# hlz0606/DH-AUG-DH-Forward-Kinematics-Model-Driven-Augmentation-for-3D-Human-Pose-Estimation

Measured on AMD Instinct MI355X. Metric: augmented poses/sec (FK+GAN step), 16-joint batch=65536, higher is better.
Workload: dtype bf16; 1 GPU; FK+Gen+D3+D2 forward; batch_per_gpu=65536, frames=1, global_batch=65536, dense_dim=256, preAngle=True, fk_dtype=f32, dense_dtype=bf16 MFMA, fp32 accumulate

## Files before the change

dh-aug-dh-forward-kinematics-model-driven-augmentation-for-3d-human-pose-estimation_amd/_lib.py:

```python
import ctypes
import os

_HERE = os.path.dirname(os.path.abspath(__file__))
LIB_PATH = os.environ.get("DHAUG_LIB", os.path.join(_HERE, "lib", "libdhaug.so"))

_vp, _i64, _i32, _f32 = ctypes.c_void_p, ctypes.c_int64, ctypes.c_int, ctypes.c_float
_u64 = ctypes.c_uint64

SIGNATURES = {
    "dhaug_fk_forward": [_vp, _vp, _vp, _vp, _i64, _i32, _vp],
    "dhaug_fk_backward": [_vp, _vp, _vp, _vp, _vp, _vp, _i64, _vp],
    "dhaug_gen_tail_forward": [_vp, _vp, _vp, _vp, _vp, _i64, _i32, _vp],
    "dhaug_gen_tail_forward_critics": [_vp, _vp, _vp, _vp, _vp, _vp, _vp, _vp, _vp, _vp, _i32, _u64, _u64, _vp, _i64, _i32, _i32, _vp],
    "dhaug_gen_tail_backward": [_vp, _vp, _vp, _vp, _vp, _i64, _i32, _vp],
    "dhaug_bone_length": [_vp, _vp, _i64, _vp],
    "dhaug_kcs_forward": [_vp, _vp, _vp, _i64, _i64, _i32, _vp],
    "dhaug_center_kcs_forward": [_vp, _vp, _vp, _i64, _i64, _i32, _vp],
    "dhaug_kcs_backward": [_vp, _vp, _vp, _i64, _i32, _vp],
    "dhaug_kcs_jvp": [_vp, _vp, _vp, _i64, _i32, _vp],
    "dhaug_world_to_camera_project": [_vp, _vp, _vp, _vp, _vp, _vp, _i64, _vp],
    "dhaug_world_to_camera_project_backward": [_vp, _vp, _vp, _vp, _vp, _vp, _vp, _i64, _vp],
    "dhaug_camera_to_world": [_vp, _vp, _vp, _vp, _i64, _vp],
    "dhaug_bone_length_swap": [_vp, _vp, _vp, _i64, _vp],
    "dhaug_project_to_2d": [_vp, _vp, _vp, _i64, _vp],
# ... 93 lines not shown
class AdamDesc(ctypes.Structure):
    _fields_ = [("off", _i64), ("len", _i64), ("nt", _vp), ("N", _i32), ("K", _i32), ("Kp", _i32), ("pad_", _i32), ("item0", _i64)]


class TnLayer(ctypes.Structure):
    _fields_ = [("A", _vp), ("lda", _i64), ("B", _vp), ("ldb", _i64), ("C", _vp), ("ldc", _i64), ("colsum_a", _vp),
                ("colsum_rows", _i64), ("M", _i64), ("N1", _i32), ("N2", _i32), ("accumulate", _i32), ("max_workgroups", _i32),
                ("planes_a", _i32), ("planes_b", _i32)]


class Block2(ctypes.Structure):
    _fields_ = [("W1", _vp), ("ldw1", _i64), ("W2", _vp), ("ldw2", _i64), ("bits1", _vp), ("bits2", _vp), ("Y1", _vp), ("ldy1", _i64),
                ("Y2", _vp), ("ldy2", _i64)]


class TopDesc(ctypes.Structure):
    _fields_ = [("seed", _vp), ("ld_seed", _i64), ("wout", _vp), ("ld_wout", _i64), ("x", _vp), ("ldx", _i64), ("m1", _vp), ("mh", _vp),
                ("m0", _vp), ("ld_m", _i64), ("w2", _vp), ("ldw2", _i64), ("w1", _vp), ("ldw1", _i64), ("wm", _vp), ("ldwm", _i64),
                ("bits0", _vp), ("bits1", _vp), ("g2", _vp), ("g1", _vp), ("g0", _vp), ("ld_g", _i64), ("gcat", _vp), ("ld_gcat", _i64),
                ("M", _i64), ("n0", _i64), ("nc", _i64), ("mask_act", _i32), ("mask_slope", _f32)]


SIGNATURES["dhaug_critic_top_backward_bf16"] = [ctypes.POINTER(TopDesc), _vp]
SIGNATURES["dhaug_critic_top_tangent_bf16"] = [ctypes.POINTER(TopDesc), _vp]
BLOCK2_MAX = 3
SIGNATURES["dhaug_gemm_block2_stack_bf16"] = [_vp, _i64, ctypes.POINTER(Block2), _i32, _i32, _f32, _i64, _vp]
TN_GROUP_MAX = 42
TN_GROUP_WORKSPACE_FLOATS = 256 * (256 * 256 + 256)
SIGNATURES["dhaug_gemm_tn_group_bf16"] = [ctypes.POINTER(TnLayer), _i32, _vp, _vp]
SIGNATURES["dhaug_pack_wfrag"] = [_vp, _i64, _vp, _i64, _i64, _i64, _vp]
SIGNATURES["dhaug_pack_wfrag_batch"] = [_vp, _i32, _vp]
SIGNATURES["dhaug_pack_wfrag_composed"] = [_vp, _i64, _vp, _vp, _i64, _vp, _vp, _vp, _i64, _i64, _i64, _i64, _vp]
SIGNATURES["dhaug_mlp_forward"] = [ctypes.POINTER(MlpUnit), _i32, _i64, _vp]
SIGNATURES["dhaug_pack_wfrag_f16x2"] = [_vp, _i64, _vp, _i64, _i64, _i64, _vp]
SIGNATURES["dhaug_pack_wfrag_f16x2_t16"] = [_vp, _i64, _vp, _i64, _i64, _i64, _vp]
SIGNATURES["dhaug_mlp_forward_x3"] = [ctypes.POINTER(MlpUnit), _i32, _i64, _vp]

EVAL_MAX_THRESHOLDS = 32
EVAL_MAX_MULTIPLICITY = 1024
EVAL_TOTALS_WORDS = 3 + EVAL_MAX_THRESHOLDS
EVAL_WORKSPACE_BYTES = 2048 * EVAL_TOTALS_WORDS * 8
LOSS_METER_WORDS = 3
POSETRAIN_WORKSPACE_BYTES = 2048 * 8

ERRORS = {-1: "DHAUG_EINVAL (bad argument)", -2: "DHAUG_EALIGN (alignment contract violated)",
          -3: "DHAUG_EUNSUPPORTED (shape not implemented)"}

_lib = None


def lib():
    global _lib
    if _lib is None:
        if not os.path.exists(LIB_PATH):
            raise RuntimeError("libdhaug.so not found at %s: build it with `python __graft_entry__.py build` "
                               "(there is no fallback path)" % LIB_PATH)
        L = ctypes.CDLL(LIB_PATH)
        L.dhaug_version.restype = ctypes.c_int
        L.dhaug_arch.restype = ctypes.c_char_p
        for name, args in SIGNATURES.items():
            fn = getattr(L, name)
            fn.argtypes = args
            fn.restype = ctypes.c_int
        if os.environ.get("DHAUG_NAN_PROPAGATION", "") in ("1", "true", "yes"):
            L.dhaug_set_nan_propagation(1)
        _lib = L
# ... 21 lines not shown
```

dh-aug-dh-forward-kinematics-model-driven-augmentation-for-3d-human-pose-estimation_amd/csrc/dhaug_mlp.hip:

```cpp
#include <cstdlib>
#include "dhaug_common.h"

namespace {

typedef short bf16x8 __attribute__((ext_vector_type(8)));
typedef short bf16x4 __attribute__((ext_vector_type(4)));
typedef float f32x16 __attribute__((ext_vector_type(16)));
typedef float f32x4 __attribute__((ext_vector_type(4)));

constexpr int MLP_BM = 128;
constexpr int MLP_MT = MLP_BM / 32;
constexpr int MLP_THREADS = 256;
constexpr int MLP_NS = 2;
constexpr int MLP_MAX_UNITS = 32;
constexpr int MLP_MAX_KSTEPS = 16;
constexpr int BUF01_PITCH = 256, BUF2_PITCH = 128;
constexpr int BUF01_BYTES = MLP_BM * BUF01_PITCH * 2;
constexpr int BUF2_BYTES = MLP_BM * BUF2_PITCH * 2;
constexpr int MLP_LDS_BYTES = 2 * BUF01_BYTES + BUF2_BYTES;

enum { U_LOAD_F32 = 0, U_LOAD_BF16 = 1, U_STORE_BF16 = 2, U_GEMM = 3 };
#if (defined(DHAUG_MLP_SAVE_TU) || defined(DHAUG_MLP_NAN_SAFE)) && !defined(SAVE_ABL_NONANSAFE)
constexpr bool NAN_SAFE_TU = true;
#else
constexpr bool NAN_SAFE_TU = false;
#endif
enum { F_OUT_F32 = 4, F_DOT_OUT = 16 };

struct Unit {
    int kind;
    int plan;
    int flags;
    int src, dst, res;
    int src2, ksteps2;
    int ksteps, N, act;
    float slope;
    int cols;
    long long ld;
    const void* g;
    const uint16_t* w;
    const uint16_t* w2;
    const float* bias;
    uint16_t* save;
    long long save_ld;
    long long save_rows;
    uint32_t* bits;
};
enum { PLAN_STACK = 1 << 13, PLAN_LEAKY = 1 << 10, PLAN_ALT = 1 << 11, PLAN_TAIL = 1 << 12, PLAN_TAIL_BF16 = 1 << 14, PLAN_OUT = 1 << 28,
       PLAN_DOT = 1 << 29, PLAN_PAIR = 1 << 30 };

struct Program {
    int nunits;
    int min_run;
    Unit u[MLP_MAX_UNITS];
};

__device__ __forceinline__ unsigned char* buf_base(unsigned char* smem, int id) {
    return smem + (id == 0 ? 0 : (id == 1 ? BUF01_BYTES : 2 * BUF01_BYTES));
}
__device__ __forceinline__ int buf_pitch_bytes(int id) { return (id == 2 ? BUF2_PITCH : BUF01_PITCH) * 2; }
__device__ __forceinline__ int chunk_off(int row, int c, int pitch_bytes) { return row * pitch_bytes + ((c ^ (row & 15)) << 4); }

__device__ __forceinline__ float act_neg(int act, float slope) {
    return act == DHAUG_ACT_RELU ? 0.0f : (act == DHAUG_ACT_LRELU ? slope : 1.0f);
}
__device__ __forceinline__ float act_fn(float v, float neg) { return fmaxf(v, v * neg); }
typedef __bf16 bf16v2 __attribute__((ext_vector_type(2)));
typedef float f32v2 __attribute__((ext_vector_type(2)));
__device__ __forceinline__ uint32_t pack_bf16x2(float a, float b) {
    f32v2 f = {a, b};
    return __builtin_bit_cast(uint32_t, __builtin_convertvector(f, bf16v2));
}

typedef short s16x2_t __attribute__((ext_vector_type(2)));
typedef uint32_t u32x4_t __attribute__((ext_vector_type(4)));
__device__ __forceinline__ uint32_t pk_relu(uint32_t packed, uint32_t lb) {
    return __builtin_bit_cast(uint32_t, __builtin_elementwise_max(__builtin_bit_cast(s16x2_t, packed), __builtin_bit_cast(s16x2_t, lb)));
}

constexpr int MLP_CH = 4;
constexpr int OUT_PITCH = 68;
typedef const Unit __attribute__((address_space(4))) * UnitPtr;
// ... 501 lines not shown
                        }
                        if (BITS && k == KS - 1) bits_store(mt - 1);
                    }
                }
                __builtin_amdgcn_sched_barrier(0);
            }
        }
        if (RESMODE == 1 || (RESMODE == 2 && has_res)) {
#pragma unroll
            for (int i = 0; i < 4; ++i) {
                acc[mt & 1][i & 1] = __builtin_amdgcn_mfma_f32_32x32x16_bf16(idl[i >> 1], rx[2 * (i & 1) + (i >> 1)], acc[mt & 1][i & 1], 0, 0, 0);
            }
            __builtin_amdgcn_sched_barrier(0);
        }
        DHAUG_LSTAMP(dbg + 1 + mt)
        DHAUG_BB_SPLIT()
    }
    if (!LEAD) quad_store(MLP_MT - 2, 28, st0, st1);
#pragma unroll
    for (int j = 0; j < 32; j += 4) {
        const uint32_t p0 = pair_pack(acc[(MLP_MT - 1) & 1], j), p1 = pair_pack(acc[(MLP_MT - 1) & 1], j + 2);
        quad_store(MLP_MT - 1, j, p0, p1);
        if (BITS) {
            bits_or(p0, j >> 1);
            bits_or(p1, (j >> 1) + 1);
        }
    }
    if (BITS) bits_store(MLP_MT - 1);
    DHAUG_LSTAMP(dbg + 5)
#pragma unroll
    for (int t = 0; t < MLP_NS; ++t) seed[t] = nseed[t];
}

__device__ __forceinline__ void tail_layer(const StackDesc& d, unsigned char* smem, int wave, int lane, const WHalf& wlo,
                                           const WHalf& whi, const f32x16 (&seed)[MLP_NS]) {
    constexpr int TILE_BYTES = 32 * BUF01_PITCH * 2;
    const int r31 = lane & 31, h = lane >> 5, x = lane & 15;
    const unsigned char* src = buf_base(smem, d.src) + wave * TILE_BYTES;
    float* st = reinterpret_cast<float*>(buf_base(smem, d.dst)) + (32 * wave + r31) * OUT_PITCH + 4 * h;
    const float neg = act_neg(d.act, d.slope);
    const int lfx = r31 * (BUF01_PITCH * 2) | ((x >> 1) << 5) | ((h ^ (x & 1)) << 4);
    bf16x8 fx[4];
#pragma unroll
    for (int k = 0; k < 3; ++k) fx[k] = *reinterpret_cast<const bf16x8*>(src + (lfx ^ (k << 5)));
    f32x16 acc[MLP_NS];
#pragma unroll
    for (int k = 0; k < MLP_MAX_KSTEPS; ++k) {
        if (k + 3 < MLP_MAX_KSTEPS) fx[(k + 3) & 3] = *reinterpret_cast<const bf16x8*>(src + (lfx ^ ((k + 3) << 5)));
#pragma unroll
        for (int t = 0; t < MLP_NS; ++t)
            acc[t] = __builtin_amdgcn_mfma_f32_32x32x16_bf16(k < 8 ? wlo[t][k & 7] : whi[t][k & 7], fx[k & 3],
                                                             k == 0 ? seed[t] : acc[t], 0, 0, 0);
    }
#pragma unroll
    for (int t = 0; t < MLP_NS; ++t)
#pragma unroll
        for (int g = 0; g < 4; ++g) {
            f32x4 v;
#pragma unroll
            for (int e = 0; e < 4; ++e) v[e] = act_fn(acc[t][4 * g + e], neg);
            *reinterpret_cast<f32x4*>(st + 32 * t + 8 * g) = v;
        }
}

__device__ __forceinline__ void tail_gemm(const StackDesc& d, unsigned char* smem, int wave, int lane, const WHalf& wlo,
                                          const WHalf& whi, const f32x16 (&seed)[MLP_NS]) {
// ... 63 lines not shown
                o.x = pack_bf16x2(act_fn(acc[mt][4 * g + 0], neg), act_fn(acc[mt][4 * g + 1], neg));
                o.y = pack_bf16x2(act_fn(acc[mt][4 * g + 2], neg), act_fn(acc[mt][4 * g + 3], neg));
                *reinterpret_cast<uint2*>(dst + chunk_off(32 * mt + r31, 4 * wave + g, pbd) + (h << 3)) = o;
            }
    }
}

struct Sweep {
    int row, c, dr, dc, q;
    __device__ __forceinline__ Sweep(int tid, int q_) : q(q_) {
        row = tid / q_; c = tid - row * q_; dr = MLP_THREADS / q_; dc = MLP_THREADS - dr * q_;
    }
    __device__ __forceinline__ void next() {
        row += dr; c += dc;
        if (c >= q) { c -= q; ++row; }
    }
};

__device__ __forceinline__ void save_image(int id, uint16_t* g, long long ld, int cols, unsigned char* smem, long long m0, long long M,
                                           int tid) {
    asm volatile("" : "+v"(tid));
#if defined(SAVE_ABL_NOSTORE)
    return;
#endif
    const unsigned char* img = buf_base(smem, id);
    const int pb = buf_pitch_bytes(id);
    for (Sweep sw(tid, cols >> 3); sw.row < MLP_BM; sw.next())
        if (m0 + sw.row < M)
            *reinterpret_cast<uint4*>(g + (m0 + sw.row) * ld + sw.c * 8) = *reinterpret_cast<const uint4*>(img + chunk_off(sw.row, sw.c, pb));
}

template <bool LEAKY, bool ALT, bool SAVE>
__device__ __forceinline__ void gemm_stack(UnitPtr lead, int lead_ks, UnitPtr first, int n, int tail, unsigned char* smem,
                                           int wave, int lane, long long m0, long long M, int tid) {
    (void)tid;
    auto save_of = [&](UnitPtr su, bool on, int& ld_bytes) -> __amdgpu_buffer_rsrc_t {
        uint16_t* base = (SAVE && on) ? su->save : nullptr;
        long long ld = (SAVE && on) ? su->save_ld : 0;
        const long long lim = (SAVE && on) ? su->save_rows : 0;
        long long rows = lim - m0 < MLP_BM ? lim - m0 : MLP_BM;
        if (rows <= 0) { rows = 0; ld = 0; base = nullptr; }
        ld_bytes = (int)(ld * 2);
#if defined(SAVE_ABL_NOSTORE) || defined(SAVE_ABL_NULLSTORES)
        base = nullptr;
#endif
        return __builtin_amdgcn_make_buffer_rsrc(base != nullptr ? base + m0 * ld : reinterpret_cast<uint16_t*>(smem), 0,
                                                 base != nullptr ? (int)(rows * ld * 2) : 0, 0x27000);
    };
    auto bits_of = [&](UnitPtr bu) -> __amdgpu_buffer_rsrc_t {
        uint32_t* base = SAVE ? bu->bits : nullptr;
        return __builtin_amdgcn_make_buffer_rsrc(base != nullptr ? base + (m0 / MLP_BM) * 1024 : reinterpret_cast<uint32_t*>(smem), 0,
                                                 base != nullptr ? 4096 : 0, 0x27000);
    };
    const int nt = n + (tail ? 1 : 0);
    StackDesc cur = stack_desc(first), nxt = stack_desc(first + (nt > 1 ? 1 : 0));
    WHalf loA, loB, hi;
    f32x16 seed[MLP_NS];
    bf16x8 idf[2];
#pragma unroll
    for (int ks2 = 0; ks2 < 2; ++ks2) {
        const int dd = (lane & 31) - 16 * ks2 - 8 * (lane >> 5);
        u32x4 v;
#pragma unroll
        for (int p2 = 0; p2 < 4; ++p2) v[p2] = (dd == 2 * p2 ? 0x3F80u : 0u) | (dd == 2 * p2 + 1 ? 0x3F800000u : 0u);
        idf[ks2] = __builtin_bit_cast(bf16x8, v);
    }
    int nold = 0;
    const __amdgpu_buffer_rsrc_t nosv = save_of(first, false, nold);
    if (lead_ks != 0) {
        const StackDesc ld = stack_desc(lead);
        load_seed(ld.bias, wave, 4, lane, seed);
        if (lead_ks == 8) {
            const WBase<8> b(ld.w, wave, 4, lane);
#pragma unroll
            for (int t = 0; t < MLP_NS; ++t)
#pragma unroll
                for (int k = 0; k < 8; ++k) loB[t][k] = b.frag(t, k);
            stack_layer<LEAKY, 0, 8, false, SAVE>(ld, cur, smem, wave, lane, loB, loA, hi, seed, idf, MLP_MAX_UNITS + 50, nosv, 0, bits_of(lead));
        } else {
            const WBase<4> b(ld.w, wave, 4, lane);
#pragma unroll
            for (int t = 0; t < MLP_NS; ++t)
#pragma unroll
                for (int k = 0; k < 4; ++k) loB[t][k] = b.frag(t, k);
            stack_layer<LEAKY, 0, 4, false, SAVE>(ld, cur, smem, wave, lane, loB, loA, hi, seed, idf, MLP_MAX_UNITS + 50, nosv, 0, bits_of(lead));
        }
        lds_barrier();
        DHAUG_LSTAMP(MLP_MAX_UNITS + 56)
    } else {
        load_seed(cur.bias, wave, 4, lane, seed);
        const WBase<> b0(cur.w, wave, 4, lane);
#pragma unroll
        for (int t = 0; t < MLP_NS; ++t)
#pragma unroll
            for (int k = 0; k < MLP_MAX_KSTEPS / 2; ++k) {
                loA[t][k] = b0.frag(t, k);
                hi[t][k] = b0.frag(t, k + 8);
            }
    }
    int l = 0;
#pragma unroll 1
    for (; l + 2 <= n; l += 2) {
// ... 247 lines not shown
    for (int i = 0; i < 2 * nw; ++i) s += st[i * MLP_BM + tid];
    static_cast<float*>(const_cast<void*>(u->g))[(m0 + tid) * u->ld] = s;
}

__device__ __forceinline__ void store_output(UnitPtr u, unsigned char* smem, long long m0, long long M, int tid) {
    const float* st = reinterpret_cast<const float*>(buf_base(smem, u->dst));
    float* out = static_cast<float*>(const_cast<void*>(u->g));
    const long long ld = u->ld;
    for (Sweep sw(tid, u->N); sw.row < MLP_BM; sw.next())
        if (m0 + sw.row < M) out[(m0 + sw.row) * ld + sw.c] = st[sw.row * OUT_PITCH + sw.c];
}

template <bool SAVE>
__global__ __launch_bounds__(MLP_THREADS, 1) void fused_mlp_kernel(Program prog, long long M) {
    extern __shared__ __attribute__((aligned(16))) unsigned char smem[];
    const int tid = threadIdx.x, lane = tid & 63;
    const int wave = __builtin_amdgcn_readfirstlane(tid >> 6);
    const long long ntiles = (M + MLP_BM - 1) / MLP_BM;
    const unsigned char __attribute__((address_space(4)))* ka =
        (const unsigned char __attribute__((address_space(4)))*)__builtin_amdgcn_kernarg_segment_ptr();
    UnitPtr units = (UnitPtr)(ka + __builtin_offsetof(Program, u));
    const int nunits = *(const int __attribute__((address_space(4)))*)(ka + __builtin_offsetof(Program, nunits));
    int hk = units->kind, hp = units->plan;
    for (long long tile = blockIdx.x; tile < ntiles; tile += gridDim.x) {
        const long long m0 = tile * MLP_BM;
        int i = 0;
#pragma unroll 1
        while (i < nunits) {
            UnitPtr u = units + i;
            const int kind = hk, plan = hp;
            int ni = i + 1;
            if (kind == U_GEMM && (plan & PLAN_STACK)) ni = i + ((plan & 15) != 0) + ((plan >> 4) & 63) + ((plan & (PLAN_TAIL | PLAN_TAIL_BF16)) ? 1 : 0);
            if (kind == U_GEMM && (plan & PLAN_PAIR)) ni = i + 2;
            {
                UnitPtr nu = units + (ni < nunits ? ni : 0);
                hk = nu->kind;
                hp = nu->plan;
            }
            DHAUG_STAMP(i)
            DHAUG_LSTAMP(MLP_MAX_UNITS + 64 + 4 * i)
            const int ui = i;
            i = ni;
            (void)ui;
            if (kind != U_GEMM) {
                if (kind == U_LOAD_BF16 && (plan & 1)) __syncthreads();
                move_unit(u, smem, m0, M, tid);
                if (kind == U_STORE_BF16) {
                    lds_barrier();
                    continue;
                }
            } else {
                if (plan & PLAN_STACK) {
                    const int lead_ks = plan & 15, run = (plan >> 4) & 63;
                    const int tail = (plan & PLAN_TAIL) ? 1 : ((plan & PLAN_TAIL_BF16) ? 2 : 0);
                    UnitPtr f0 = u + (lead_ks != 0), tu = f0 + run;
                    if ((plan & PLAN_LEAKY) || NAN_SAFE_TU) gemm_stack<true, false, SAVE>(u, lead_ks, f0, run, tail, smem, wave, lane, m0, M, tid);
                    else if (plan & PLAN_ALT) gemm_stack<false, true, SAVE>(u, lead_ks, f0, run, tail, smem, wave, lane, m0, M, tid);
                    else gemm_stack<false, false, SAVE>(u, lead_ks, f0, run, tail, smem, wave, lane, m0, M, tid);
                    lds_barrier();
                    if (SAVE) {
                        UnitPtr lu = tu - 1;
                        if (lu->save != nullptr) save_image(lu->dst, lu->save, lu->save_ld, (lu->N + 15) & ~15, smem, m0, lu->save_rows, tid);
                        if (tail == 2 && tu->save != nullptr)
                            save_image(tu->dst, tu->save, tu->save_ld, (tu->N + 15) & ~15, smem, m0, tu->save_rows, tid);
                    }
                    if (tail == 1) {
                        store_output(tu, smem, m0, M, tid);
                        lds_barrier();
                    }

                    continue;
                }
                const int nslices = (plan >> 24) & 15, dbg = MLP_MAX_UNITS + 64 + 4 * ui;
                if (plan & PLAN_PAIR) {
                    gemm_pair(u, u + 1, smem, wave, lane, dbg);
                    if ((u + 1)->flags & F_DOT_OUT) {
                        lds_barrier();
                        dot_output(u + 1, smem, m0, M, tid);
                    }
                    lds_barrier();
                    DHAUG_LSTAMP(dbg + 7)
                    continue;
                }
#define DHAUG_SHAPES(NS)                                                                   \
    switch ((plan >> 16) & 255) {                               \
        case 1 * 16 + 1: gemm_single<1, 1, NS>(u, smem, wave, lane, dbg); break;                 \
        case 2 * 16 + 2: gemm_single<2, 2, NS>(u, smem, wave, lane, dbg); break;                 \
        case 2 * 16 + 1: gemm_single<2, 1, NS>(u, smem, wave, lane, dbg); break;                 \
        case 4 * 16 + 4: gemm_single<4, 4, NS>(u, smem, wave, lane, dbg); break;                 \
        case 4 * 16 + 2: gemm_single<4, 2, NS>(u, smem, wave, lane, dbg); break;                 \
        case 8 * 16 + 4: gemm_single<8, 4, NS>(u, smem, wave, lane, dbg); break;                 \
// ... 60 lines not shown
        for (int m = 0; m < d.K2; ++m) c = fma((double)a[m], (double)d.bias2[m], c);
        s += c;
    }
    return (float)s;
}

__device__ __forceinline__ void pack_desc(const dhaug_wfrag_desc& d) {
    const long long total = (long long)8 * d.ksteps * 64 * 8;
    uint16_t* dst = static_cast<uint16_t*>(d.dst);
    for (long long i = (long long)blockIdx.x * 256 + threadIdx.x; i < total; i += (long long)gridDim.x * 256) {
        const int j = (int)(i & 7), lane = (int)((i >> 3) & 63);
        const long long blk = i >> 9;
        const int ks = (int)(blk % d.ksteps), sl = (int)(blk / d.ksteps);
        const int n = 32 * sl + (lane & 31), k = 16 * ks + 8 * (lane >> 5) + j;
        dst[i] = (n < d.N && k < d.K) ? dhaug_f32_to_bf16(wfrag_elem(d, n, k)) : (uint16_t)0;
    }
    if (blockIdx.x == 0) {
        const int t = threadIdx.x;
        if (d.bias_dst != nullptr) d.bias_dst[t] = t < d.N ? wfrag_bias(d, t) : 0.0f;
        if (d.dot_dst != nullptr) {
            d.dot_dst[t] = t < d.K ? dhaug_bf16_to_f32(dhaug_f32_to_bf16(wfrag_elem(d, 0, t))) : 0.0f;
            if (t == 0) d.dot_dst[256] = wfrag_bias(d, 0);
        }
    }
}

__global__ __launch_bounds__(256) void pack_wfrag_batch_kernel(const dhaug_wfrag_desc* __restrict__ descs) {
    const dhaug_wfrag_desc d = descs[blockIdx.y];
    pack_desc(d);
}

__global__ __launch_bounds__(256) void pack_wfrag_desc_kernel(const dhaug_wfrag_desc d) { pack_desc(d); }

int plan_unit(const Program& p, int i) {
    const Unit* U = p.u;
    const Unit& u = U[i];
    if (u.kind != U_GEMM) {
        int parks = 0;
        for (int j = 0; j < p.nunits; ++j) parks |= U[j].kind == U_STORE_BF16;
        return u.kind == U_LOAD_BF16 ? parks : 0;
    }
    const bool wide = u.ksteps2 == 0 && u.N > 224 && !(u.flags & (F_OUT_F32 | F_DOT_OUT)) && u.src < 2 && u.dst < 2;
    const int ks4 = (u.ksteps + 3) & ~3;
    const int lead_ks = (wide && u.res < 0 && ks4 <= 8) ? ks4 : 0;
    const int i0 = i + (lead_ks != 0);
    int run = 0, leaky = lead_ks != 0 && u.act == DHAUG_ACT_LRELU, alt = 1;
    while (i0 + run < p.nunits && U[i0 + run].kind == U_GEMM && U[i0 + run].ksteps == 16 && U[i0 + run].ksteps2 == 0 &&
           U[i0 + run].N > 224 && !(U[i0 + run].flags & (F_OUT_F32 | F_DOT_OUT)) && U[i0 + run].src < 2 && U[i0 + run].dst < 2 &&
           U[i0 + run].res < 2) {
        leaky |= U[i0 + run].act == DHAUG_ACT_LRELU;
        alt &= (U[i0 + run].res >= 0) == ((run & 1) == 1);
        ++run;
    }
    if (run < p.min_run || run > 63) {
        const int c1 = (u.ksteps + 3) / 4, c2 = (u.ksteps2 + 3) / 4;
        auto narrow = [&](const Unit& v) {
            return v.kind == U_GEMM && v.ksteps2 == 0 && v.ksteps > 4 && v.ksteps <= 8 && v.N > 96 && v.N <= 128 && !(v.flags & F_OUT_F32) &&
                   v.save == nullptr;
        };
        const bool second = i > 0 && (U[i - 1].plan & PLAN_PAIR) && U[i - 1].kind == U_GEMM && !(U[i - 1].plan & PLAN_STACK);
        const bool pair = !second && i + 1 < p.nunits && narrow(u) && !(u.flags & F_DOT_OUT) && narrow(U[i + 1]) &&
                          !getenv("DHAUG_MLP_NOPAIR");
        return (((c1 + c2) * 16 + c1) << 16) | (((u.N + 31) >> 5) << 24) | ((u.flags & F_OUT_F32) ? PLAN_OUT : 0) |
               ((u.flags & F_DOT_OUT) ? PLAN_DOT : 0) | (pair ? PLAN_PAIR : 0);
    }
    const Unit* tu = U + i0 + run;
    const bool tail = i0 + run < p.nunits && tu->kind == U_GEMM && (tu->flags & F_OUT_F32) && tu->ksteps == 16 &&
                      tu->ksteps2 == 0 && tu->N <= 64 && tu->src < 2 && tu->dst < 2 && tu->res < 0;
    const bool tail2 = !tail && i0 + run < p.nunits && tu->kind == U_GEMM && !(tu->flags & (F_OUT_F32 | F_DOT_OUT)) &&
                       tu->ksteps == 16 && tu->ksteps2 == 0 && tu->N <= 128 && tu->src < 2 && tu->res != tu->src &&
                       !getenv("DHAUG_MLP_NOTAIL2");
    return PLAN_STACK | lead_ks | (run << 4) | (leaky ? PLAN_LEAKY : 0) | ((!leaky && alt && !(run & 1)) ? PLAN_ALT : 0) |
           (tail ? PLAN_TAIL : 0) | (tail2 ? PLAN_TAIL_BF16 : 0);
// ... 12 lines not shown
    const int ksteps = (int)((K + 63) / 64) * 4, nslices = 8;
    DHAUG_CHECK(ksteps <= MLP_MAX_KSTEPS && N <= 256, DHAUG_EUNSUPPORTED);
    const long long total = (long long)nslices * ksteps * 512;
    long long blocks = (total + 255) / 256;
    if (blocks > 1024) blocks = 1024;
    hipLaunchKernelGGL(pack_wfrag_kernel, dim3((unsigned)blocks), dim3(256), 0, (hipStream_t)stream, W, (long long)ldw, dst,
                       (int)N, (int)K, (int)k0, ksteps, nslices);
    return dhaug_launch_status();
}

int dhaug_pack_wfrag_batch(const dhaug_wfrag_desc* descs_device, int n, void* stream) {
    DHAUG_CHECK(n >= 0, DHAUG_EINVAL);
    if (n == 0) return DHAUG_OK;
    DHAUG_CHECK_PTR(descs_device);
    hipLaunchKernelGGL(pack_wfrag_batch_kernel, dim3(64, (unsigned)n), dim3(256), 0, (hipStream_t)stream, descs_device);
    return dhaug_launch_status();
}

int dhaug_pack_wfrag_composed(const float* Wa, int64_t ldwa, const float* bias_a, const float* Wb, int64_t ldwb, const float* bias_b,
                              uint16_t* dst, float* bias_dst, int64_t N, int64_t Ki, int64_t K, int64_t k0, void* stream) {
    DHAUG_CHECK(N >= 1 && Ki >= 1 && K >= 1 && k0 >= 0 && ldwa >= Ki && ldwb >= k0 + K, DHAUG_EINVAL);
    DHAUG_CHECK_PTR(Wa); DHAUG_CHECK_PTR(Wb); DHAUG_CHECK_PTR(dst);
    DHAUG_CHECK(dhaug_aligned16(dst), DHAUG_EALIGN);
    const int ksteps = (int)((K + 63) / 64) * 4;
    DHAUG_CHECK(ksteps <= MLP_MAX_KSTEPS && N <= 256 && Ki <= (1 << 20), DHAUG_EUNSUPPORTED);
    dhaug_wfrag_desc d = {};
    d.W = Wa; d.ldw = ldwa; d.dst = dst; d.bias = bias_a; d.bias_dst = bias_dst; d.dot_dst = nullptr;
    d.N = (int32_t)N; d.K = (int32_t)K; d.k0 = (int32_t)k0; d.ksteps = ksteps;
    d.W2 = Wb; d.bias2 = bias_b; d.ldw2 = ldwb; d.K2 = (int32_t)Ki;
    hipLaunchKernelGGL(pack_wfrag_desc_kernel, dim3(64), dim3(256), 0, (hipStream_t)stream, d);
    return dhaug_launch_status();
}

int dhaug_mlp_forward(const dhaug_mlp_unit* units, int nunits, int64_t M, void* stream) {
    DHAUG_CHECK(nunits >= 1 && nunits <= MLP_MAX_UNITS && M >= 0, DHAUG_EINVAL);
    DHAUG_CHECK_PTR(units);
    if (M == 0) return DHAUG_OK;
    Program prog;
    prog.nunits = nunits;
    prog.min_run = getenv("DHAUG_MLP_NOSTACK") ? 1 << 20 : 2;
    bool any_save = false;
    for (int i = 0; i < nunits; ++i) {
        const dhaug_mlp_unit& s = units[i];
        Unit& u = prog.u[i];
        u.kind = s.kind; u.flags = s.flags; u.src = s.src; u.dst = s.dst; u.res = s.res;
        u.src2 = s.src2; u.ksteps2 = s.ksteps2;
        u.ksteps = s.ksteps; u.N = s.n; u.act = s.act; u.slope = s.slope; u.cols = s.cols; u.ld = s.ld;
        if (dhaug_nan_propagation_ && s.kind == U_GEMM && s.act == DHAUG_ACT_RELU) { u.act = DHAUG_ACT_LRELU; u.slope = 0.0f; }
        u.g = s.g; u.w = static_cast<const uint16_t*>(s.w); u.w2 = static_cast<const uint16_t*>(s.w2); u.bias = s.bias;
        u.save = static_cast<uint16_t*>(s.save); u.save_ld = s.save_ld;
        u.save_rows = s.save_rows == 0 ? M : (s.save_rows < 0 ? 0 : (s.save_rows < M ? s.save_rows : M));
        u.bits = static_cast<uint32_t*>(s.bits);
        DHAUG_CHECK(u.kind >= U_LOAD_F32 && u.kind <= U_GEMM, DHAUG_EINVAL);
        if (u.bits != nullptr) {
            DHAUG_CHECK(u.kind == U_GEMM && u.save != nullptr && u.N > 224, DHAUG_EINVAL);
            DHAUG_CHECK(dhaug_aligned16(u.bits), DHAUG_EALIGN);
        }
        if (u.save != nullptr) {
            DHAUG_CHECK(u.kind == U_GEMM && !(u.flags & (F_OUT_F32 | F_DOT_OUT)), DHAUG_EINVAL);
            DHAUG_CHECK(dhaug_aligned16(u.save) && u.save_ld % 8 == 0 && u.save_ld >= ((u.N + 15) & ~15), DHAUG_EALIGN);
            any_save = true;
        }
        auto okbuf = [](int b) { return b >= 0 && b <= 2; };
        auto pitch = [](int b) { return b == 2 ? BUF2_PITCH : BUF01_PITCH; };
        if (u.kind == U_GEMM) {
            DHAUG_CHECK(okbuf(u.src) && u.ksteps >= 1 && u.ksteps <= MLP_MAX_KSTEPS && u.N >= 1 && u.N <= 256, DHAUG_EUNSUPPORTED);
            DHAUG_CHECK(((u.ksteps + 3) / 4) * 64 <= pitch(u.src), DHAUG_EUNSUPPORTED);
            DHAUG_CHECK(u.w != nullptr && dhaug_aligned16(u.w), DHAUG_EALIGN);
            DHAUG_CHECK(u.bias != nullptr && dhaug_aligned16(u.bias), DHAUG_EALIGN);
            DHAUG_CHECK(u.ksteps2 >= 0 && u.ksteps2 <= MLP_MAX_KSTEPS, DHAUG_EUNSUPPORTED);
            if (u.ksteps2 > 0) {
                DHAUG_CHECK(okbuf(u.src2) && ((u.ksteps2 + 3) / 4) * 64 <= pitch(u.src2), DHAUG_EUNSUPPORTED);
                DHAUG_CHECK(u.ksteps % 4 == 0, DHAUG_EUNSUPPORTED);
                DHAUG_CHECK(u.w2 != nullptr && dhaug_aligned16(u.w2), DHAUG_EALIGN);
            }
            {
                const int c1 = (u.ksteps + 3) / 4, c2 = (u.ksteps2 + 3) / 4, sh = (c1 + c2) * 16 + c1;
                const bool ok = sh == 17 || sh == 34 || sh == 33 || sh == 68 || sh == 66 || sh == 132;
                DHAUG_CHECK(ok, DHAUG_EUNSUPPORTED);
            }
            if (u.flags & F_DOT_OUT) {
                DHAUG_CHECK(u.ksteps <= 8 && u.N <= 128, DHAUG_EUNSUPPORTED);
                DHAUG_CHECK(!(u.flags & F_OUT_F32) && u.ksteps2 == 0 && u.g != nullptr && u.ld >= 1 && u.w2 != nullptr &&
                            dhaug_aligned16(u.w2) && (u.dst == 0 || u.dst == 1) && u.dst != u.src && u.dst != u.res, DHAUG_EINVAL);
            }
            if (u.flags & F_OUT_F32) {
                DHAUG_CHECK(u.g != nullptr && u.ld >= u.N && u.N <= 64, DHAUG_EUNSUPPORTED);
                DHAUG_CHECK((u.dst == 0 || u.dst == 1) && u.dst != u.src && (u.ksteps2 == 0 || u.dst != u.src2), DHAUG_EINVAL);
                DHAUG_CHECK(u.res < 0, DHAUG_EINVAL);
            } else {
                DHAUG_CHECK(okbuf(u.dst) && u.dst != u.src && (u.ksteps2 == 0 || u.dst != u.src2), DHAUG_EINVAL);
                DHAUG_CHECK(((u.N + 31) / 32) * 32 <= pitch(u.dst), DHAUG_EUNSUPPORTED);
                DHAUG_CHECK(u.res < 0 || (okbuf(u.res) && u.res != u.src && (u.ksteps2 == 0 || u.res != u.src2)), DHAUG_EINVAL);
            }
        } else {
            const int b = u.kind == U_STORE_BF16 ? u.src : u.dst;
            DHAUG_CHECK(okbuf(b) && u.g != nullptr && u.cols >= 8 && ((u.cols + 63) & ~63) <= pitch(b), DHAUG_EINVAL);
            DHAUG_CHECK(u.cols % 8 == 0 && u.ld >= u.cols && dhaug_aligned16(u.g), DHAUG_EALIGN);
            DHAUG_CHECK(u.kind == U_LOAD_F32 ? (u.ld % 4 == 0) : (u.ld % 8 == 0), DHAUG_EALIGN);
        }
    }
    for (int i = 0; i < prog.nunits; ++i) prog.u[i].plan = plan_unit(prog, i);
    {
        bool in_run[MLP_MAX_UNITS] = {};
        for (int i = 0; i < prog.nunits;) {
            const int plan = prog.u[i].plan;
            if (prog.u[i].kind == U_GEMM && (plan & PLAN_STACK)) {
                const int lead = (plan & 15) != 0, run = (plan >> 4) & 63;
                for (int j = 0; j < lead + run; ++j) in_run[i + j] = true;
                i += lead + run + ((plan & (PLAN_TAIL | PLAN_TAIL_BF16)) ? 1 : 0);
            } else {
                ++i;
            }
        }
        for (int i = 0; i < prog.nunits; ++i) DHAUG_CHECK(prog.u[i].bits == nullptr || in_run[i], DHAUG_EUNSUPPORTED);
    }
    const long long ntiles = (M + MLP_BM - 1) / MLP_BM;
    const unsigned grid = dhaug_persistent_grid(ntiles);
    if (any_save) return dhaug_mlp_launch_save_(&prog, (long long)M, grid, stream);
    if (const int rc = dhaug_dynamic_lds<fused_mlp_kernel<false>>(MLP_LDS_BYTES)) return rc;
    hipLaunchKernelGGL(fused_mlp_kernel<false>, dim3(grid), dim3(MLP_THREADS), MLP_LDS_BYTES, (hipStream_t)stream, prog, (long long)M);
    return dhaug_launch_status();
}

}

#endif

#ifdef DHAUG_MLP_TIMING
extern "C" int dhaug_debug_mlp_stamps(long long* out, int n) {
    return (int)hipMemcpyFromSymbol(out, HIP_SYMBOL(g_mlp_stamps), sizeof(long long) * (n < 6 * MLP_MAX_UNITS + 69 ? n : 6 * MLP_MAX_UNITS + 69));
}
#endif
```

include/dhaug.h:

```cpp
#ifndef DHAUG_H
#define DHAUG_H

#include <stdint.h>

#ifdef __cplusplus
extern "C" {
#endif

#define DHAUG_VERSION 100

#define DHAUG_OK             0
#define DHAUG_EINVAL        -1
#define DHAUG_EALIGN        -2
#define DHAUG_EUNSUPPORTED  -3

#define DHAUG_ACT_NONE   0
#define DHAUG_ACT_RELU   1
#define DHAUG_ACT_LRELU  2

int dhaug_version(void);
const char* dhaug_arch(void);


int dhaug_fk_forward(const float* angles, const float* bone_len, const float* root, float* out,
// ... 223 lines not shown
    int cols;
    int64_t ld;
    const void* g;
    const void* w;
    const void* w2;
    const float* bias;
    void* save;
    int64_t save_ld;
    void* bits;
    int64_t save_rows;
} dhaug_mlp_unit;

typedef struct dhaug_wfrag_desc {
    const float* W;
    int64_t ldw;
    void* dst;
    const float* bias;
    float* bias_dst;
    float* dot_dst;
    int32_t N, K, k0, ksteps;
    const float* W2;
    const float* bias2;
    int64_t ldw2;
    int32_t K2;
    int32_t pad_;
} dhaug_wfrag_desc;
int dhaug_pack_wfrag_batch(const dhaug_wfrag_desc* descs_device, int n, void* stream);

int dhaug_pack_wfrag_composed(const float* Wa, int64_t ldwa, const float* bias_a, const float* Wb, int64_t ldwb, const float* bias_b,
                              uint16_t* dst, float* bias_dst, int64_t N, int64_t Ki, int64_t K, int64_t k0, void* stream);

int dhaug_mlp_forward(const dhaug_mlp_unit* units, int nunits, int64_t M, void* stream);

int dhaug_pack_wfrag_f16x2(const float* W, int64_t ldw, uint16_t* dst, int64_t N, int64_t K, int64_t k0, void* stream);
#define DHAUG_MLP_F_T16      32
int dhaug_pack_wfrag_f16x2_t16(const float* W, int64_t ldw, uint16_t* dst, int64_t N, int64_t K, int64_t k0, void* stream);
#define DHAUG_MLP_X3_WORKSPACE_BYTES (2 * 256 * 4 * 64 * 128 * 4)
int dhaug_mlp_forward_x3(const dhaug_mlp_unit* units, int nunits, int64_t M, void* stream);


int dhaug_colsum_f32(const float* src, int64_t ld, float* dst, int64_t M, int64_t N, int accumulate,
                     void* stream);
int dhaug_colsum_bf16(const uint16_t* src, int64_t ld, float* dst, int64_t M, int64_t N, int accumulate,
                      void* stream);

int dhaug_act_backward_bf16(const uint16_t* g, int64_t ld_g, const uint16_t* y, int64_t ld_y,
                            uint16_t* dst, int64_t ld_dst, int64_t M, int64_t N, int act, float slope,
                            void* stream);

int dhaug_act_backward_f32(const float* g, const float* y, float* dst, int64_t n, int act, float slope,
                           void* stream);

int dhaug_adam_step(float* param, const float* grad, float* exp_avg, float* exp_avg_sq, int64_t n,
                    float lr, float beta1, float beta2, float eps, int step, float grad_scale, void* stream);

int dhaug_adam_step_dev(float* param, const float* grad, float* exp_avg, float* exp_avg_sq, int64_t n,
                        float lr, float beta1, float beta2, float eps, const int* step_dev, float grad_scale, void* stream);
int dhaug_counter_add(int* counter, int value, void* stream);

typedef struct dhaug_repack_desc {
    const float* W;
    void* nt;
    void* nn;
    int N, K, Kp, Np;
} dhaug_repack_desc;
int dhaug_repack_weights(const dhaug_repack_desc* descs_device, int nparams, void* stream);
// ... 99 lines not shown
```

Baseline: 306.2 million poses/s.

## Feed narrow bf16 lead GEMM operand directly from global memory into registers

Adds a plan flag that fuses a narrow (32 or 48 column) bf16 load unit with the following stacked lead GEMM. The lead GEMM's B operand is then read from global memory straight into registers through buffer loads, skipping the LDS staging copy and its barrier. The planner only enables this when no later unit reads the staged buffer and no save path is active. A plan-query entry point and an env opt-out are also added. In exchange the lead operand occupies more VGPRs, and the planner logic becomes more complex.

```diff
diff --git a/dh-aug-dh-forward-kinematics-model-driven-augmentation-for-3d-human-pose-estimation_amd/_lib.py b/dh-aug-dh-forward-kinematics-model-driven-augmentation-for-3d-human-pose-estimation_amd/_lib.py
--- a/dh-aug-dh-forward-kinematics-model-driven-augmentation-for-3d-human-pose-estimation_amd/_lib.py
+++ b/dh-aug-dh-forward-kinematics-model-driven-augmentation-for-3d-human-pose-estimation_amd/_lib.py
@@ -149,6 +149,8 @@
 SIGNATURES["dhaug_pack_wfrag_batch"] = [_vp, _i32, _vp]
 SIGNATURES["dhaug_pack_wfrag_composed"] = [_vp, _i64, _vp, _vp, _i64, _vp, _vp, _vp, _i64, _i64, _i64, _i64, _vp]
 SIGNATURES["dhaug_mlp_forward"] = [ctypes.POINTER(MlpUnit), _i32, _i64, _vp]
+SIGNATURES["dhaug_mlp_plan"] = [ctypes.POINTER(MlpUnit), _i32, _i64, ctypes.POINTER(ctypes.c_int32)]
+MLP_PLAN_STACK, MLP_PLAN_LEADG = 1 << 13, 1 << 15
 SIGNATURES["dhaug_pack_wfrag_f16x2"] = [_vp, _i64, _vp, _i64, _i64, _i64, _vp]
 SIGNATURES["dhaug_pack_wfrag_f16x2_t16"] = [_vp, _i64, _vp, _i64, _i64, _i64, _vp]
 SIGNATURES["dhaug_mlp_forward_x3"] = [ctypes.POINTER(MlpUnit), _i32, _i64, _vp]
diff --git a/dh-aug-dh-forward-kinematics-model-driven-augmentation-for-3d-human-pose-estimation_amd/csrc/dhaug_mlp.hip b/dh-aug-dh-forward-kinematics-model-driven-augmentation-for-3d-human-pose-estimation_amd/csrc/dhaug_mlp.hip
--- a/dh-aug-dh-forward-kinematics-model-driven-augmentation-for-3d-human-pose-estimation_amd/csrc/dhaug_mlp.hip
+++ b/dh-aug-dh-forward-kinematics-model-driven-augmentation-for-3d-human-pose-estimation_amd/csrc/dhaug_mlp.hip
@@ -48,6 +48,7 @@
 };
 enum { PLAN_STACK = 1 << 13, PLAN_LEAKY = 1 << 10, PLAN_ALT = 1 << 11, PLAN_TAIL = 1 << 12, PLAN_TAIL_BF16 = 1 << 14, PLAN_OUT = 1 << 28,
        PLAN_DOT = 1 << 29, PLAN_PAIR = 1 << 30 };
+enum { PLAN_LEADG = 1 << 15 };
 
 struct Program {
     int nunits;
@@ -615,6 +616,114 @@
     for (int t = 0; t < MLP_NS; ++t) seed[t] = nseed[t];
 }
 
+template <int KS>
+__device__ __forceinline__ void lead_operand(UnitPtr lu, long long m0, long long M, int lane, bf16x8 (&gx)[MLP_MT][KS]) {
+    const long long ld = lu->ld, left = M - m0;
+    const int rows = left < MLP_BM ? (int)left : MLP_BM, ldb = (int)ld * 2;
+    const __amdgpu_buffer_rsrc_t rs = __builtin_amdgcn_make_buffer_rsrc(
+        const_cast<uint16_t*>(static_cast<const uint16_t*>(lu->g)) + m0 * ld, 0, (rows - 1) * ldb + 32 * KS, 0x27000);
+    const int off = (lane & 31) * ldb + ((lane >> 5) << 4);
+#pragma unroll
+    for (int mt = 0; mt < MLP_MT; ++mt)
+#pragma unroll
+        for (int k = 0; k < KS; ++k)
+            gx[mt][k] = __builtin_bit_cast(bf16x8, __builtin_amdgcn_raw_buffer_load_b128(rs, off + 32 * mt * ldb + 32 * k, 0, 0));
+}
+
+template <bool LEAKY, int KS>
+__device__ __forceinline__ void stack_lead_global(const StackDesc& d, const StackDesc& nd, unsigned char* smem, int wave, int lane,
+                                                  const bf16x8 (&gx)[MLP_MT][KS], const WHalf& wl, WHalf& nlo, WHalf& whi,
+                                                  f32x16 (&seed)[MLP_NS], int dbg) {
+    DHAUG_LSTAMP(dbg)
+    static_assert(KS == 2 || KS == 3, "32 or 48 columns");
+    constexpr int TILE_BYTES = 32 * BUF01_PITCH * 2, NM = MLP_NS * KS;
+    const int r31 = lane & 31, h = lane >> 5, x = lane & 15;
+    f32x16 nseed[MLP_NS];
+    const int ns0 = nd.narrow ? 0 : wave, nss = nd.narrow ? 1 : 4;
+    const WBase<> nb(nd.w, ns0, nss, lane);
+    const float neg = act_neg(d.act, d.slope);
+    const uint32_t lb = d.act == DHAUG_ACT_RELU ? 0u : 0x80008000u;
+    const int lep = r31 * (BUF01_PITCH * 2) | (((4 * wave) ^ x) << 4) | (h << 3);
+    typedef const unsigned char __attribute__((address_space(3))) * LdsPtr;
+    typedef unsigned char __attribute__((address_space(3))) * LdsWPtr;
+    uint32_t wa[4];
+    {
+        const uint32_t db = (uint32_t)(uintptr_t)(LdsPtr)buf_base(smem, d.dst);
+#pragma unroll
+        for (int g = 0; g < 4; ++g) {
+            wa[g] = db + (uint32_t)(lep ^ (g << 4));
+            asm volatile("" : "+v"(wa[g]));
+        }
+    }
+    f32x16 acc[2][MLP_NS];
+    auto pair_pack = [&](const f32x16 (&a)[MLP_NS], int j) -> uint32_t {
+        const int t = j >> 4, g = (j >> 2) & 3, e = j & 3;
+        const float v0 = a[t][4 * g + e], v1 = a[t][4 * g + e + 1];
+        if (!LEAKY)
+            return __builtin_bit_cast(uint32_t, __builtin_elementwise_max(__builtin_bit_cast(s16x2, pack_bf16x2(v0, v1)),
+                                                                          __builtin_bit_cast(s16x2, lb)));
+        return pack_bf16x2(act_fn(v0, neg), act_fn(v1, neg));
+    };
+    auto quad_store = [&](int mt, int j) {
+        const int t = j >> 4, g = (j >> 2) & 3;
+        typedef uint32_t u32x2 __attribute__((ext_vector_type(2)));
+        const u32x2 oo = {pair_pack(acc[mt & 1], j), pair_pack(acc[mt & 1], j + 2)};
+#ifdef ABL_NOWRITE
+        asm volatile("" :: "v"(oo));
+#else
+        *reinterpret_cast<u32x2 __attribute__((address_space(3)))*>((LdsWPtr)(uintptr_t)wa[g] + (t << 8) + mt * TILE_BYTES) = oo;
+#endif
+    };
+#pragma unroll
+    for (int mt = 0; mt < MLP_MT; ++mt) {
+#pragma unroll
+        for (int i = 0; i < NM; ++i) {
+            const int k = i / MLP_NS, t = i % MLP_NS;
+            acc[mt & 1][t] = __builtin_amdgcn_mfma_f32_32x32x16_bf16(wl[t][k], gx[mt][k], k == 0 ? seed[t] : acc[mt & 1][t], 0, 0, 0);
+            __builtin_amdgcn_sched_barrier(0);
+            if (mt == MLP_MT - 1 && i == 0) load_seed(nd.bias, ns0, nss, lane, nseed);
+#ifndef ABL_NOWLOAD
+            if (mt == 1 || mt == 2) {
+#pragma unroll
+                for (int f = 0; f < 16; ++f) {
+                    if (f < 16 * i / NM || f >= 16 * (i + 1) / NM) continue;
+                    if (mt == 1) nlo[f >> 3][f & 7] = nb.frag(f >> 3, f & 7);
+                    else whi[f >> 3][f & 7] = nb.frag(f >> 3, 8 + (f & 7));
+                }
+            }
+#endif
+            if (mt > 0) {
+#pragma unroll
+                for (int q = 0; q < 8; ++q)
+                    if (q >= 8 * i / NM && q < 8 * (i + 1) / NM) quad_store(mt - 1, 4 * q);
+            }
+            __builtin_amdgcn_sched_barrier(0);
+        }
+        DHAUG_LSTAMP(dbg + 1 + mt)
+        DHAUG_BB_SPLIT()
+    }
+#pragma unroll
+    for (int q = 0; q < 8; ++q) quad_store(MLP_MT - 1, 4 * q);
+    DHAUG_LSTAMP(dbg + 5)
+#pragma unroll
+    for (int t = 0; t < MLP_NS; ++t) seed[t] = nseed[t];
+}
+
+template <bool LEAKY, int KS>
+__device__ __forceinline__ void lead_from_global(UnitPtr gl, const StackDesc& ld, const StackDesc& cur, unsigned char* smem, int wave,
+                                                 int lane, long long m0, long long M, WHalf& loA, WHalf& loB, WHalf& hi,
+                                                 f32x16 (&seed)[MLP_NS]) {
+    bf16x8 gx[MLP_MT][KS];
+    lead_operand<KS>(gl, m0, M, lane, gx);
+    load_seed(ld.bias, wave, 4, lane, seed);
+    const WBase<4> b(ld.w, wave, 4, lane);
+#pragma unroll
+    for (int t = 0; t < MLP_NS; ++t)
+#pragma unroll
+        for (int k = 0; k < KS; ++k) loB[t][k] = b.frag(t, k);
+    stack_lead_global<LEAKY, KS>(ld, cur, smem, wave, lane, gx, loB, loA, hi, seed, MLP_MAX_UNITS + 50);
+}
+
 __device__ __forceinline__ void tail_layer(const StackDesc& d, unsigned char* smem, int wave, int lane, const WHalf& wlo,
                                            const WHalf& whi, const f32x16 (&seed)[MLP_NS]) {
     constexpr int TILE_BYTES = 32 * BUF01_PITCH * 2;
@@ -744,7 +853,7 @@
 
 template <bool LEAKY, bool ALT, bool SAVE>
 __device__ __forceinline__ void gemm_stack(UnitPtr lead, int lead_ks, UnitPtr first, int n, int tail, unsigned char* smem,
-                                           int wave, int lane, long long m0, long long M, int tid) {
+                                           int wave, int lane, long long m0, long long M, int tid, UnitPtr gl = nullptr, int gks = 0) {
     (void)tid;
     auto save_of = [&](UnitPtr su, bool on, int& ld_bytes) -> __amdgpu_buffer_rsrc_t {
         uint16_t* base = (SAVE && on) ? su->save : nullptr;
@@ -779,7 +888,13 @@
     }
     int nold = 0;
     const __amdgpu_buffer_rsrc_t nosv = save_of(first, false, nold);
-    if (lead_ks != 0) {
+    if (!SAVE && gks != 0) {
+        const StackDesc ld = stack_desc(lead);
+        if (gks == 2) lead_from_global<LEAKY, 2>(gl, ld, cur, smem, wave, lane, m0, M, loA, loB, hi, seed);
+        else lead_from_global<LEAKY, 3>(gl, ld, cur, smem, wave, lane, m0, M, loA, loB, hi, seed);
+        lds_barrier();
+        DHAUG_LSTAMP(MLP_MAX_UNITS + 56)
+    } else if (lead_ks != 0) {
         const StackDesc ld = stack_desc(lead);
         load_seed(ld.bias, wave, 4, lane, seed);
         if (lead_ks == 8) {
@@ -1093,6 +1208,8 @@
             int ni = i + 1;
             if (kind == U_GEMM && (plan & PLAN_STACK)) ni = i + ((plan & 15) != 0) + ((plan >> 4) & 63) + ((plan & (PLAN_TAIL | PLAN_TAIL_BF16)) ? 1 : 0);
             if (kind == U_GEMM && (plan & PLAN_PAIR)) ni = i + 2;
+            const bool leadg = !SAVE && kind == U_LOAD_BF16 && (plan & PLAN_LEADG);
+            if (leadg) ni = i + 2 + ((plan >> 4) & 63) + ((plan & (PLAN_TAIL | PLAN_TAIL_BF16)) ? 1 : 0);
             {
                 UnitPtr nu = units + (ni < nunits ? ni : 0);
                 hk = nu->kind;
@@ -1103,7 +1220,7 @@
             const int ui = i;
             i = ni;
             (void)ui;
-            if (kind != U_GEMM) {
+            if (kind != U_GEMM && !leadg) {
                 if (kind == U_LOAD_BF16 && (plan & 1)) __syncthreads();
                 move_unit(u, smem, m0, M, tid);
                 if (kind == U_STORE_BF16) {
@@ -1112,12 +1229,12 @@
                 }
             } else {
                 if (plan & PLAN_STACK) {
-                    const int lead_ks = plan & 15, run = (plan >> 4) & 63;
+                    const int gks = leadg ? (plan & 15) : 0, lead_ks = leadg ? 4 : (plan & 15), run = (plan >> 4) & 63;
                     const int tail = (plan & PLAN_TAIL) ? 1 : ((plan & PLAN_TAIL_BF16) ? 2 : 0);
-                    UnitPtr f0 = u + (lead_ks != 0), tu = f0 + run;
-                    if ((plan & PLAN_LEAKY) || NAN_SAFE_TU) gemm_stack<true, false, SAVE>(u, lead_ks, f0, run, tail, smem, wave, lane, m0, M, tid);
-                    else if (plan & PLAN_ALT) gemm_stack<false, true, SAVE>(u, lead_ks, f0, run, tail, smem, wave, lane, m0, M, tid);
-                    else gemm_stack<false, false, SAVE>(u, lead_ks, f0, run, tail, smem, wave, lane, m0, M, tid);
+                    UnitPtr lu = u + (leadg ? 1 : 0), f0 = lu + (lead_ks != 0), tu = f0 + run;
+                    if ((plan & PLAN_LEAKY) || NAN_SAFE_TU) gemm_stack<true, false, SAVE>(lu, lead_ks, f0, run, tail, smem, wave, lane, m0, M, tid, u, gks);
+                    else if (plan & PLAN_ALT) gemm_stack<false, true, SAVE>(lu, lead_ks, f0, run, tail, smem, wave, lane, m0, M, tid, u, gks);
+                    else gemm_stack<false, false, SAVE>(lu, lead_ks, f0, run, tail, smem, wave, lane, m0, M, tid, u, gks);
                     lds_barrier();
                     if (SAVE) {
                         UnitPtr lu = tu - 1;
@@ -1244,13 +1361,28 @@
 
 __global__ __launch_bounds__(256) void pack_wfrag_desc_kernel(const dhaug_wfrag_desc d) { pack_desc(d); }
 
-int plan_unit(const Program& p, int i) {
+int plan_unit(const Program& p, int i, bool leadg = false) {
     const Unit* U = p.u;
     const Unit& u = U[i];
     if (u.kind != U_GEMM) {
         int parks = 0;
         for (int j = 0; j < p.nunits; ++j) parks |= U[j].kind == U_STORE_BF16;
-        return u.kind == U_LOAD_BF16 ? parks : 0;
+        if (u.kind != U_LOAD_BF16) return 0;
+        if (!leadg || parks || getenv("DHAUG_MLP_NOLEADG") || (u.cols != 32 && u.cols != 48) || u.ld > (1 << 20) || i + 1 >= p.nunits)
+            return parks;
+        const Unit& l = U[i + 1];
+        if (l.kind != U_GEMM || l.src != u.dst) return parks;
+        const int sp = plan_unit(p, i + 1);
+        if (!(sp & PLAN_STACK) || (sp & 15) != 4) return parks;
+        const int b = u.dst, run_end = i + 2 + ((sp >> 4) & 63);
+        for (int j = i + 2; j < p.nunits; ++j) {
+            const Unit& v = U[j];
+            if (v.kind == U_STORE_BF16 ? v.src == b
+                                       : (v.kind == U_GEMM && (v.src == b || (v.ksteps2 > 0 && v.src2 == b) || v.res == b)))
+                return parks;
+            if (v.dst == b && (v.kind != U_GEMM || j < run_end)) break;
+        }
+        return (sp & ~15) | (u.cols >> 4) | PLAN_LEADG;
     }
     const bool wide = u.ksteps2 == 0 && u.N > 224 && !(u.flags & (F_OUT_F32 | F_DOT_OUT)) && u.src < 2 && u.dst < 2;
     const int ks4 = (u.ksteps + 3) & ~3;
@@ -1329,14 +1461,14 @@
     return dhaug_launch_status();
 }
 
-int dhaug_mlp_forward(const dhaug_mlp_unit* units, int nunits, int64_t M, void* stream) {
+}
+
+static int mlp_prepare(const dhaug_mlp_unit* units, int nunits, int64_t M, Program& prog, bool& any_save) {
     DHAUG_CHECK(nunits >= 1 && nunits <= MLP_MAX_UNITS && M >= 0, DHAUG_EINVAL);
     DHAUG_CHECK_PTR(units);
-    if (M == 0) return DHAUG_OK;
-    Program prog;
     prog.nunits = nunits;
     prog.min_run = getenv("DHAUG_MLP_NOSTACK") ? 1 << 20 : 2;
-    bool any_save = false;
+    any_save = false;
     for (int i = 0; i < nunits; ++i) {
         const dhaug_mlp_unit& s = units[i];
         Unit& u = prog.u[i];
@@ -1397,7 +1529,7 @@
             DHAUG_CHECK(u.kind == U_LOAD_F32 ? (u.ld % 4 == 0) : (u.ld % 8 == 0), DHAUG_EALIGN);
         }
     }
-    for (int i = 0; i < prog.nunits; ++i) prog.u[i].plan = plan_unit(prog, i);
+    for (int i = 0; i < prog.nunits; ++i) prog.u[i].plan = plan_unit(prog, i, !any_save);
     {
         bool in_run[MLP_MAX_UNITS] = {};
         for (int i = 0; i < prog.nunits;) {
@@ -1412,6 +1544,27 @@
         }
         for (int i = 0; i < prog.nunits; ++i) DHAUG_CHECK(prog.u[i].bits == nullptr || in_run[i], DHAUG_EUNSUPPORTED);
     }
+    return DHAUG_OK;
+}
+
+extern "C" {
+
+int dhaug_mlp_plan(const dhaug_mlp_unit* units, int nunits, int64_t M, int32_t* plans_out) {
+    DHAUG_CHECK_PTR(plans_out);
+    Program prog;
+    bool any_save;
+    if (const int rc = mlp_prepare(units, nunits, M, prog, any_save)) return rc;
+    for (int i = 0; i < nunits; ++i) plans_out[i] = prog.u[i].plan;
+    return DHAUG_OK;
+}
+
+int dhaug_mlp_forward(const dhaug_mlp_unit* units, int nunits, int64_t M, void* stream) {
+    DHAUG_CHECK(nunits >= 1 && nunits <= MLP_MAX_UNITS && M >= 0, DHAUG_EINVAL);
+    DHAUG_CHECK_PTR(units);
+    if (M == 0) return DHAUG_OK;
+    Program prog;
+    bool any_save;
+    if (const int rc = mlp_prepare(units, nunits, M, prog, any_save)) return rc;
     const long long ntiles = (M + MLP_BM - 1) / MLP_BM;
     const unsigned grid = dhaug_persistent_grid(ntiles);
     if (any_save) return dhaug_mlp_launch_save_(&prog, (long long)M, grid, stream);
diff --git a/include/dhaug.h b/include/dhaug.h
--- a/include/dhaug.h
+++ b/include/dhaug.h
@@ -279,6 +279,10 @@
 
 int dhaug_mlp_forward(const dhaug_mlp_unit* units, int nunits, int64_t M, void* stream);
 
+#define DHAUG_MLP_PLAN_STACK  (1 << 13)
+#define DHAUG_MLP_PLAN_LEADG  (1 << 15)
+int dhaug_mlp_plan(const dhaug_mlp_unit* units, int nunits, int64_t M, int32_t* plans_out);
+
 int dhaug_pack_wfrag_f16x2(const float* W, int64_t ldw, uint16_t* dst, int64_t N, int64_t K, int64_t k0, void* stream);
 #define DHAUG_MLP_F_T16      32
 int dhaug_pack_wfrag_f16x2_t16(const float* W, int64_t ldw, uint16_t* dst, int64_t N, int64_t K, int64_t k0, void* stream);
```

Measured after the change: 311.6 million poses/s (median of 6 runs). +1.8%, better.
